# ma921/SOBER

Measured on AMD Instinct MI355X. Metric: recombination-step candidates/sec (N_rec=100000, N_nys=500, d=10, batch=100), higher is better.
Workload: dtype f64

## Files before the change

sober_amd/csrc/chol.hip:

```cpp
#include "common.hpp"
#include "internal.hpp"

namespace sober {

constexpr int CH_NB = 32;
constexpr int CH_T = 512;
constexpr int CH_LDPP = CH_NB + 4;
constexpr int CH_MAXN = 536;

typedef double ch_double4 __attribute__((ext_vector_type(4)));

constexpr int CH_G = 4;
__device__ double ch_sink[CH_T];
#ifdef CM_STAMPS
__device__ double ch_dbg[2];
#endif

__device__ __forceinline__ double ch_rdlane(double v, int l) {
    return __hiloint2double(__builtin_amdgcn_readlane(__double2hiint(v), l),
                            __builtin_amdgcn_readlane(__double2loint(v), l));
}

template <int NC>
__device__ __attribute__((noinline)) void ch_diag_block_n(double* __restrict__ D, double* __restrict__ Xs, double* __restrict__ s_dinv,
                                              int* __restrict__ s_fail_p, double* __restrict__ s_minp_p, int nb, int kb,
                                              int lane, double* __restrict__ xout) {
    constexpr int LDP = CH_NB + 1;
    int& s_fail = *s_fail_p;
    double& s_minp = *s_minp_p;

            const int i = lane & (CH_NB - 1);
            const bool xh = lane >= CH_NB;
            double v[CH_NB];
#ifdef CM_STAMPS
            const long long dbg0 = wall_clock64();
#endif
#pragma unroll
            for (int c = 0; c < CH_NB; ++c) {
                double dv = D[i * LDP + c];
                asm volatile("" : "+v"(dv));
                v[c] = (xh | (i >= nb)) ? ((c == i) ? 1.0 : 0.0) : dv;
            }
            const bool xw = xout != nullptr && xh;
            double* xo = xw ? xout + (size_t)(kb / CH_NB) * CH_NB * CH_NB : ch_sink;
            const int xo_ld = xw ? CH_NB : 0, xo_i = xw ? i : lane;
            double* const o_base = xh ? Xs + i : D + i * LDP;
            const int o_step = xh ? LDP : 1;
            int fail = 0;
            double minp = s_minp;
#pragma unroll
            for (int j = 0; j < NC; ++j) {
                const double djj = ch_rdlane(v[j], j);
                const bool live = (j < nb) & (fail == 0);
                minp = live ? fmin(minp, djj) : minp;
                fail = (live & !(djj > 0.0)) ? kb + j + 1 : fail;
                double rinv = __builtin_amdgcn_rsq(djj);
                {
                    double h = 0.5 * rinv, e = fma(-(djj * rinv), h, 0.5);
                    rinv = fma(rinv, e, rinv);
                    h = 0.5 * rinv; e = fma(-(djj * rinv), h, 0.5);
                    rinv = fma(rinv, e, rinv);
                }
                double l = djj * rinv;
                l = fma(fma(-l, l, djj), 0.5 * rinv, l);
                const double sc = v[j] * rinv;
                v[j] = xh ? sc : ((i == j) ? l : ((i > j) ? sc : 0.0));
                o_base[j * o_step] = v[j];
                xo[j * xo_ld + xo_i] = v[j];
#pragma unroll
                for (int c = j + 1; c < NC; ++c) {
                    const double lcj = ch_rdlane(v[j], c);
                    v[c] = fma(-v[j], lcj, v[c]);
                }
            }
#pragma unroll
            for (int j = NC; j < CH_NB; ++j) { o_base[j * o_step] = v[j]; xo[j * xo_ld + xo_i] = v[j]; }
            if (lane == 0) { s_fail = fail; s_minp = minp; }
#ifdef CM_STAMPS
            if (lane == 0) { ch_dbg[0] = (double)(wall_clock64() - dbg0); ch_dbg[1] = 0.0; }
#endif
        }

__device__ __forceinline__ void ch_diag_block(double* __restrict__ D, double* __restrict__ Xs, double* __restrict__ s_dinv,
                                              int* __restrict__ s_fail_p, double* __restrict__ s_minp_p, int nb, int kb,
                                              int lane, double* __restrict__ xout) {
    if (nb <= 8) ch_diag_block_n<8>(D, Xs, s_dinv, s_fail_p, s_minp_p, nb, kb, lane, xout);
    else if (nb <= 16) ch_diag_block_n<16>(D, Xs, s_dinv, s_fail_p, s_minp_p, nb, kb, lane, xout);
    else ch_diag_block_n<CH_NB>(D, Xs, s_dinv, s_fail_p, s_minp_p, nb, kb, lane, xout);
}

constexpr int CH_SMALLN = 120;
template <bool SMALL>
__global__ __launch_bounds__(CH_T) void k_chol(double* __restrict__ A, int n, int ld, double shift,
                                              int32_t* __restrict__ info, double* __restrict__ min_pivot,
                                              const double* __restrict__ src, int lds_src,
                                              const double* __restrict__ shifts, double* __restrict__ xout,
                                              double* __restrict__ ratio_out) {
    extern __shared__ double lds[];
    if (src != nullptr) {
        A += (size_t)blockIdx.x * n * ld;
        info += blockIdx.x;
        if (min_pivot) min_pivot += blockIdx.x;
        shift = shifts[blockIdx.x];
        for (int i = threadIdx.x >> 6; i < n; i += CH_T / 64)
            for (int j = threadIdx.x & 63; j <= i; j += 64) A[(size_t)i * ld + j] = src[(size_t)i * lds_src + j];
        __threadfence_block();
        __syncthreads();
    }
    constexpr int LDP = CH_NB + 1;
    double* D = lds;
    double* Xs = lds + CH_NB * LDP;
    constexpr int LDPP = CH_LDPP;
    double* P = lds + 2 * CH_NB * LDP;
    double* const A_glob = A;
    const int ld_glob = ld;
    double* As = nullptr;
    if constexpr (SMALL) {
        As = P + (size_t)(n > CH_NB ? n - CH_NB : 0) * LDPP;
    }
    __shared__ int s_fail;
    __shared__ double s_minp;
    __shared__ double s_dinv[CH_NB];
    const int tid = threadIdx.x, lane = tid & 63, wave = tid >> 6;
    const int li = lane & 15, lk = lane >> 4;
    if (tid == 0) { s_fail = 0; s_minp = __builtin_inf(); }
    __shared__ double s_dm[CH_T / 64];
    if (ratio_out != nullptr) {
        double dl = -__builtin_inf();
        for (int i = tid; i < n; i += CH_T) dl = fmax(dl, A_glob[(size_t)i * ld_glob + i] + shift);
#pragma unroll
        for (int o = 32; o > 0; o >>= 1) dl = fmax(dl, __shfl_xor(dl, o, 64));
        if (lane == 0) s_dm[wave] = dl;
    }
    __syncthreads();
    bool ahead0 = false;
    if constexpr (SMALL) {
        const int nb0 = min(CH_NB, n);
#pragma unroll
        for (int t = tid; t < CH_NB * CH_NB; t += CH_T) {
            const int i = t >> 5, j = t & 31;
            double v = (i < nb0 && j <= i) ? A_glob[(size_t)i * ld_glob + j] : 0.0;
            if (i == j && i < nb0) v += shift;
            D[i * LDP + j] = v;
        }
        __syncthreads();
        if (wave == 0) {
            ch_diag_block(D, Xs, s_dinv, &s_fail, &s_minp, nb0, 0, lane, xout);
        } else {
            for (int i = wave - 1; i < n; i += CH_T / 64 - 1)
                for (int j = lane; j <= i; j += 64) As[i * (n + 1) + j] = A_glob[(size_t)i * ld_glob + j];
        }
        A = As;
        ld = n + 1;
        __syncthreads();
        ahead0 = true;
    }
#ifdef CH_STAMPS
    long long st_t[5] = {0, 0, 0, 0, 0}, st_last = wall_clock64();
#define CH_STAMP(K) { const long long now_ = wall_clock64(); st_t[K] += now_ - st_last; st_last = now_; }
#else
#define CH_STAMP(K)
#endif

    bool ahead = ahead0;
    for (int kb = 0; kb < n; kb += CH_NB) {
        const int nb = min(CH_NB, n - kb);
        const int nr = n - kb - nb;
        if (!ahead) {
#pragma unroll
            for (int t = tid; t < CH_NB * CH_NB; t += CH_T) {
                const int i = t >> 5, j = t & 31;
                double v = (i < nb && j <= i) ? A[(size_t)(kb + i) * ld + kb + j] : 0.0;
                if (i == j && i < nb) v += shift;
                D[i * LDP + j] = v;
            }
            __syncthreads();
            CH_STAMP(0)
            if (wave == 0) ch_diag_block(D, Xs, s_dinv, &s_fail, &s_minp, nb, kb, lane, xout);
            __syncthreads();
            CH_STAMP(1)
        }
        if (s_fail != 0) break;
#pragma unroll
        for (int t = tid; t < CH_NB * CH_NB; t += CH_T) {
            const int i = t >> 5, j = t & 31;
            if (i < nb && j <= i) A[(size_t)(kb + i) * ld + kb + j] = D[i * LDP + j];
        }
        if (nr == 0) break;
        {
            const int ntile = (nr + 15) / 16;
            double af[8], an[8];
            if (wave < ntile) {
                const double* arow = A + (size_t)(kb + nb + min(wave * 16 + li, nr - 1)) * ld + kb;
#pragma unroll
                for (int u = 0; u < 8; ++u) af[u] = arow[min(4 * u + lk, nb - 1)];
            }
            for (int t = wave; t < ntile; t += CH_T / 64) {
                const int r0 = t * 16;
                {
                    const int tn = min(t + CH_T / 64, ntile - 1);
                    const double* arow = A + (size_t)(kb + nb + min(tn * 16 + li, nr - 1)) * ld + kb;
#pragma unroll
                    for (int u = 0; u < 8; ++u) an[u] = arow[min(4 * u + lk, nb - 1)];
                }
                ch_double4 acc0 = (ch_double4){0.0, 0.0, 0.0, 0.0}, acc1 = acc0;
#pragma unroll
                for (int u = 0; u < 8; ++u) {
                    const int k = 4 * u + lk;
                    const double a = (k < nb) ? af[u] : 0.0;
                    acc0 = __builtin_amdgcn_mfma_f64_16x16x4f64(a, Xs[li * LDP + k], acc0, 0, 0, 0);
                    acc1 = __builtin_amdgcn_mfma_f64_16x16x4f64(a, Xs[(16 + li) * LDP + k], acc1, 0, 0, 0);
                }
#pragma unroll
                for (int r = 0; r < 4; ++r) {
                    const int row = r0 + lk + 4 * r;
                    if (row < nr) {
                        P[row * LDPP + li] = acc0[r];
                        P[row * LDPP + 16 + li] = acc1[r];
                    }
                }
#pragma unroll
                for (int u = 0; u < 8; ++u) af[u] = an[u];
            }
        }
        __syncthreads();
        CH_STAMP(2)
        for (int r = tid >> 5; r < nr; r += CH_T / 32) {
            const int j = tid & 31;
            if (j < nb) A[(size_t)(kb + nb + r) * ld + kb + j] = P[r * LDPP + j];
        }
        {
            const int nt = (nr + 15) / 16;
            const int wv = __builtin_amdgcn_readfirstlane(wave);
            const bool look = nt * (nt + 1) / 2 >= 8;
            const int t_step = look ? (wv == 0 ? 1 : CH_T / 64 - 1) : CH_T / 64;
            const int nt_mine = (look && wv == 0) ? min(nt, 2) : nt;
            int ntr = 0, ntc = look ? (wv == 0 ? 0 : 2 + wv) : wv;
            while (ntc > ntr) { ntc -= ntr + 1; ++ntr; }
            int tr[CH_G], tc[CH_G], trn[CH_G], tcn[CH_G];
            double cv[CH_G][4], cn[CH_G][4];
            double* const a22 = A + (size_t)(kb + nb) * ld + kb + nb;
// ... 277 lines not shown
                unsigned v = 1u;
                if (jf <= jmax) v = cm_poll(rs, fbase + CM_OFF_FP + 4 * (k * CM_G + o));
                if (v != 1u) s_flag = 0xffu;
            }
        };
        auto gather = [&](int t0, int nthr) {
            for (int cb = k + 1; cb <= jmax; cb += 8)
                for (int gi = t0; gi < CH_NB * CH_NB / 2; gi += nthr) {
                    const int i = gi >> 4, j = (gi & 15) * 2;
                    ch_u32x4 v[8];
#pragma unroll
                    for (int q = 0; q < 8; ++q) {
                        const int c = cb + q, row = min(CH_NB * c + i, n - 1);
                        if (c <= jmax && cm_owner(c) != g)
                            v[q] = __builtin_amdgcn_raw_buffer_load_b128(ra, (unsigned)(((size_t)row * ld + kb + j) * 8), 0, 16);
                    }
#pragma unroll
                    for (int q = 0; q < 8; ++q) {
                        const int c = cb + q, row = CH_NB * c + i;
                        if (c <= jmax && cm_owner(c) != g && row < n) {
                            double* pr = P + (size_t)(row - kb - CH_NB) * LDPP + j;
                            pr[0] = __hiloint2double((int)v[q].y, (int)v[q].x);
                            pr[1] = __hiloint2double((int)v[q].w, (int)v[q].z);
                        }
                    }
                }
        };
        auto walk = [&](int cs0, int wslot, int nwalk) {
            int cs = cs0, ct = wslot;
                int tr[CH_G], tc[CH_G], trn[CH_G], tcn[CH_G];
                double cv[CH_G][4], cn[CH_G][4];
#define CM_TAKE(R, C)                                                                           \
                { while (cs < n_strips && ct > strip_r0(cs) / 16) { ct -= strip_r0(cs) / 16 + 1; ++cs; }   \
                  R = cs < n_strips ? strip_r0(cs) : -1; C = cs < n_strips ? 16 * ct : 0; ct += nwalk; }
#define CM_LOAD(DST, R, C)                                                                      \
                _Pragma("unroll") for (int e = 0; e < 4; ++e)                                   \
                    DST[e] = a22[(size_t)min(max(R, 0) + lk + 4 * e, nr - 1) * ld + min((C) + li, nr - 1)];
#pragma unroll
                for (int q = 0; q < CH_G; ++q) { CM_TAKE(tr[q], tc[q]) CM_LOAD(cv[q], tr[q], tc[q]) }
                while (tr[0] >= 0) {
#pragma unroll
                    for (int q = 0; q < CH_G; ++q) { CM_TAKE(trn[q], tcn[q]) CM_LOAD(cn[q], trn[q], tcn[q]) }
                    ch_double4 acc[CH_G][2];
#pragma unroll
                    for (int q = 0; q < CH_G; ++q) {
                        acc[q][0] = (ch_double4){0.0, 0.0, 0.0, 0.0};
                        acc[q][1] = acc[q][0];
                        const int pa = min(max(tr[q], 0) + li, nr - 1), pb = min(tc[q] + li, nr - 1);
#pragma unroll
                        for (int u = 0; u < 8; u += 2) {
                            acc[q][0] = __builtin_amdgcn_mfma_f64_16x16x4f64(P[pa * LDPP + 4 * u + lk], P[pb * LDPP + 4 * u + lk], acc[q][0], 0, 0, 0);
                            acc[q][1] = __builtin_amdgcn_mfma_f64_16x16x4f64(P[pa * LDPP + 4 * u + 4 + lk], P[pb * LDPP + 4 * u + 4 + lk], acc[q][1], 0, 0, 0);
                        }
                    }
#pragma unroll
                    for (int q = 0; q < CH_G; ++q)
#pragma unroll
                        for (int e = 0; e < 4; ++e) {
                            const int row = tr[q] + lk + 4 * e, col = tc[q] + li;
                            double* dst = (tr[q] >= 0 && row < nr && col <= row) ? a22 + (size_t)row * ld + col : ch_sink + tid;
                            *dst = cv[q][e] - (acc[q][0][e] + acc[q][1][e]);
                        }
#pragma unroll
                    for (int q = 0; q < CH_G; ++q) {
                        tr[q] = trn[q]; tc[q] = tcn[q];
#pragma unroll
                        for (int e = 0; e < 4; ++e) cv[q][e] = cn[q][e];
                    }
                }
#undef CM_TAKE
#undef CM_LOAD
        };
        if (!look) {
            poll_others(tid);
            __syncthreads();
            CM_STAMP(2)
            if (s_flag != 0xffu) gather(tid, CH_T);
            __syncthreads();
            CM_STAMP(3)
            if (s_flag != 0xffu) walk(0, wave, CH_T / 64);
        } else if (wave == 0) {
            __builtin_amdgcn_s_setprio(3);
            const int R0[3] = {0, 16, 16}, C0[3] = {0, 0, 16};
            double cv[3][4];
#pragma unroll
            for (int q = 0; q < 3; ++q)
#pragma unroll
                for (int e = 0; e < 4; ++e)
                    cv[q][e] = a22[(size_t)min(R0[q] + lk + 4 * e, nr - 1) * ld + min(C0[q] + li, nr - 1)];
#pragma unroll
            for (int q = 0; q < 3; ++q) {
                ch_double4 acc0 = (ch_double4){0.0, 0.0, 0.0, 0.0}, acc1 = acc0;
                const int pa = min(R0[q] + li, nr - 1), pb = min(C0[q] + li, nr - 1);
#pragma unroll
                for (int u = 0; u < 8; u += 2) {
                    acc0 = __builtin_amdgcn_mfma_f64_16x16x4f64(P[pa * LDPP + 4 * u + lk], P[pb * LDPP + 4 * u + lk], acc0, 0, 0, 0);
                    acc1 = __builtin_amdgcn_mfma_f64_16x16x4f64(P[pa * LDPP + 4 * u + 4 + lk], P[pb * LDPP + 4 * u + 4 + lk], acc1, 0, 0, 0);
                }
#pragma unroll
                for (int e = 0; e < 4; ++e) {
                    const int row = R0[q] + lk + 4 * e, col = C0[q] + li;
                    double* dst = (row < nr && col <= row) ? a22 + (size_t)row * ld + col : ch_sink + tid;
                    *dst = cv[q][e] - (acc0[e] + acc1[e]);
                }
            }
            __builtin_amdgcn_s_waitcnt(0);
            const int kb2 = kb + CH_NB, nb2 = min(CH_NB, n - kb2);
#pragma unroll
            for (int t = lane; t < CH_NB * CH_NB; t += 64) {
                const int i = t >> 5, j = t & 31;
                double v = (i < nb2 && j <= i) ? A[(size_t)(kb2 + i) * ld + kb2 + j] : 0.0;
                if (i == j && i < nb2) v += shift;
                D[i * LDP + j] = v;
            }
            __builtin_amdgcn_wave_barrier();
            ch_diag_block(D, Xs, s_dinv, &s_fail, &s_minp, nb2, kb2, lane, nullptr);
            __builtin_amdgcn_s_setprio(0);
        } else {
            if (wave == 1) poll_others(lane);
            sub_barrier();
            if (s_flag != 0xffu) gather(tid - 64, CH_T - 64);
            sub_barrier();
            if (s_flag != 0xffu) walk(2, wave - 1, CH_T / 64 - 1);
        }
        CM_STAMP(4)
        ahead = look;
        __threadfence_block();
        __syncthreads();
        CM_STAMP(5)
        if (s_flag == 0xffu) {
            if (tid == 0) {
                __builtin_amdgcn_raw_buffer_store_b32(1, rs, CM_OFF_ERR, 0, 16);
                info[rung] = CM_INFO_EXCHANGE;
            }
            break;
        }
    }
#ifdef CM_STAMPS
    if (tid == 0 && n >= 480) { for (int q = 0; q < 6; ++q) A[(size_t)g * ld + 400 + q] = (double)cs_t[q]; A[(size_t)g * ld + 410] = ch_dbg[0]; A[(size_t)g * ld + 411] = ch_dbg[1]; }
#endif
    if (verdict >= 0 && tid == 0) {
        double mp = s_minp;
        for (int q = 0; q < verdict; ++q) {
            const unsigned lo = (unsigned)__builtin_amdgcn_raw_buffer_load_b32(rs, fbase + CM_OFF_MP + 8 * q, 0, 16);
            const unsigned hi = (unsigned)__builtin_amdgcn_raw_buffer_load_b32(rs, fbase + CM_OFF_MP + 8 * q + 4, 0, 16);
            mp = fmin(mp, __hiloint2double((int)hi, (int)lo));
        }
        info[rung] = s_fail;
        if (min_pivot) min_pivot[rung] = mp;
    }
}

constexpr int TB_WAVES = 2;
__global__ __launch_bounds__(TB_WAVES * 64) void k_trsm_blocks(const double* __restrict__ Y, int64_t m, int q, int ldy,
                                                              const double* __restrict__ L, int ldl,
                                                              const double* __restrict__ Xinv,
                                                              double* __restrict__ Q, int ldq) {
    extern __shared__ double tb_lds[];
    const int lane = threadIdx.x & 63, wave = threadIdx.x >> 6;
    const int li = lane & 15, lk = lane >> 4;
    const int qpad = ((q + 31) / 32) * 32, LS = qpad + 4;
    double* stash = tb_lds + (size_t)wave * (16 * LS + 16 * 36);
    double* tbuf = stash + 16 * LS;
    const int64_t R0 = ((int64_t)blockIdx.x * TB_WAVES + wave) * 16;
    if (R0 >= m) return;
    const int nblk = qpad / 32;
    for (int jb = 0; jb < nblk; ++jb) {
        const int c0 = 32 * jb;
        ch_double4 acc[2];
#pragma unroll
        for (int jt = 0; jt < 2; ++jt)
#pragma unroll
            for (int r = 0; r < 4; ++r) {
                const int64_t row = min(R0 + lk + 4 * r, m - 1);
                const int col = c0 + 16 * jt + li;
                const double v = Y[row * ldy + min(col, q - 1)];
                acc[jt][r] = (col < q) ? v : 0.0;
            }
        for (int kb = 0; kb < jb; ++kb) {
#pragma unroll
            for (int u = 0; u < 8; ++u) {
                const int kc = 32 * kb + 4 * u + lk;
                const double a = -stash[li * LS + kc];
#pragma unroll
                for (int jt = 0; jt < 2; ++jt) {
                    const int lr = c0 + 16 * jt + li;
                    const double b = L[(size_t)min(lr, q - 1) * ldl + kc];
                    acc[jt] = __builtin_amdgcn_mfma_f64_16x16x4f64(a, (lr < q) ? b : 0.0, acc[jt], 0, 0, 0);
                }
            }
        }
#pragma unroll
        for (int jt = 0; jt < 2; ++jt)
#pragma unroll
            for (int r = 0; r < 4; ++r) tbuf[(lk + 4 * r) * 36 + 16 * jt + li] = acc[jt][r];
        __builtin_amdgcn_wave_barrier();
        const double* X = Xinv + (size_t)jb * 32 * 32;
        ch_double4 out[2] = {(ch_double4){0.0, 0.0, 0.0, 0.0}, (ch_double4){0.0, 0.0, 0.0, 0.0}};
#pragma unroll
        for (int u = 0; u < 8; ++u) {
            const double a = tbuf[li * 36 + 4 * u + lk];
#pragma unroll
            for (int jt = 0; jt < 2; ++jt)
                out[jt] = __builtin_amdgcn_mfma_f64_16x16x4f64(a, X[(16 * jt + li) * 32 + 4 * u + lk], out[jt], 0, 0, 0);
        }
        __builtin_amdgcn_wave_barrier();
#pragma unroll
        for (int jt = 0; jt < 2; ++jt)
#pragma unroll
            for (int r = 0; r < 4; ++r) {
                const int64_t row = R0 + lk + 4 * r;
                const int col = c0 + 16 * jt + li;
                stash[(lk + 4 * r) * LS + col] = out[jt][r];
                if (row < m && col < q) Q[row * ldq + col] = out[jt][r];
            }
        __builtin_amdgcn_wave_barrier();
    }
}

__global__ __launch_bounds__(256) void k_abs_sym(const double* __restrict__ C, int n, int ld,
                                                 double* __restrict__ out, int ldo, int32_t* __restrict__ flag,
                                                 unsigned long long* __restrict__ dmax_bits) {
    __shared__ double tm[32][33];
    const int tx = threadIdx.x & 31, ty = threadIdx.x >> 5;
    const int i0 = blockIdx.y * 32, j0 = blockIdx.x * 32;
    for (int r = ty; r < 32; r += 8) {
        const int i = j0 + r, j = i0 + tx;
        tm[r][tx] = (i < n && j < n) ? C[(size_t)i * ld + j] : 0.0;
    }
    __syncthreads();
    bool asym = false;
    const double big = 1.7976931348623157e308;
    for (int r = ty; r < 32; r += 8) {
        const int i = i0 + r, j = j0 + tx;
        if (i < n && j < n) {
            double a = C[(size_t)i * ld + j], b = tm[tx][r];
            asym |= !(a == b);
            a = (a != a) ? 0.0 : fmin(fmax(a, -big), big);
            b = (b != b) ? 0.0 : fmin(fmax(b, -big), big);
            const double v = sqrt(a * b);
            out[(size_t)i * ldo + j] = v;
            if (dmax_bits != nullptr && i == j) atomicMax(dmax_bits, (unsigned long long)__double_as_longlong(v));
        }
    }
    if (__syncthreads_or(asym) && threadIdx.x == 0) atomicOr(flag, 1);
}

__global__ void k_jitter_ladder(double* __restrict__ A, int n, int ld, int k) {
    const int i = blockIdx.x * blockDim.x + threadIdx.x;
    if (i >= n) return;
    double d = A[(size_t)i * ld + i], jit = 1e-5;
    for (int t = 0; t < k; ++t) { d = __dadd_rn(d, jit); jit = __dmul_rn(jit, 2.0); }
    A[(size_t)i * ld + i] = d;
}

__global__ void k_jitter_ladder_auto(double* __restrict__ A, int n, int ld, const int32_t* __restrict__ info,
                                     int n_rungs, int32_t* __restrict__ k_out) {
    const int j = blockIdx.x * blockDim.x + threadIdx.x, i = blockIdx.y;
    int k = 0;
    while (k < n_rungs && info[k] != 0) ++k;
    if (i == 0 && j == 0) *k_out = k;
    if (j >= n) return;
    if (i == j) {
        double d = A[(size_t)i * ld + i], jit = 1e-5;
        for (int t = 0; t < k; ++t) { d = __dadd_rn(d, jit); jit = __dmul_rn(jit, 2.0); }
        A[(size_t)i * ld + i] = d;
    } else if (k == n_rungs) {
        A[(size_t)i * ld + j] = 0.0;
    }
}

}

namespace sober {
__global__ void k_probe_mc_init(uint32_t* __restrict__ ws, int64_t n_words, int32_t* __restrict__ info, int n_info, int32_t value,
                                uint32_t* __restrict__ pre, int64_t n_pre) {
    const int64_t t = (int64_t)blockIdx.x * blockDim.x + threadIdx.x;
    if (t < n_words) ws[t] = 0u;
    if (pre != nullptr) {
        const int64_t i0 = (uint32_t*)info - pre;
        if (t < n_pre && !(t >= i0 && t < i0 + n_info)) pre[t] = 0u;
    }
    if (t < n_info) info[t] = value;
}
}

namespace sober {
constexpr int CB_MAXN = 2048;
constexpr int CB_TILE = 64;

__global__ __launch_bounds__(256) void k_cb_init(double* __restrict__ work, int n, const double* __restrict__ src, int ld_src,
                                                 int32_t* __restrict__ info, double* __restrict__ min_pivot, int n_rungs) {
    const int i = blockIdx.x, rung = blockIdx.y;
    double* A = work + (size_t)rung * n * n;
    for (int c = threadIdx.x; c <= i; c += 256) A[(size_t)i * n + c] = src[(size_t)i * ld_src + c];
    if (i == 0 && threadIdx.x == 0) { info[rung] = 0; if (min_pivot) min_pivot[rung] = __builtin_inf(); }
}

__global__ __launch_bounds__(64) void k_cb_diag(double* __restrict__ work, int n, int kb, const double* __restrict__ shifts,
                                                double* __restrict__ xinv, int32_t* __restrict__ info,
                                                double* __restrict__ min_pivot) {
    constexpr int LDP = CH_NB + 1;
    __shared__ double D[CH_NB * LDP], Xs[CH_NB * LDP], s_dinv[CH_NB];
    __shared__ int s_fail;
    __shared__ double s_minp;
    const int rung = blockIdx.x, lane = threadIdx.x;
    double* A = work + (size_t)rung * n * n;
    const int nb = min(CH_NB, n - kb);
    const double shift = shifts[rung];
#pragma unroll
    for (int t = lane; t < CH_NB * CH_NB; t += 64) {
        const int i = t >> 5, j = t & 31;
        double v = (i < nb && j <= i) ? A[(size_t)(kb + i) * n + kb + j] : 0.0;
        if (i == j && i < nb) v += shift;
        D[i * LDP + j] = v;
    }
    if (lane == 0) { s_fail = 0; s_minp = __builtin_inf(); }
// ... 13 lines not shown
    constexpr int LDP = CH_NB + 1, LDPP = CH_LDPP;
    __shared__ double Xs[CH_NB * LDP], Pr[CB_TILE * LDPP], Pc[CB_TILE * LDPP];
    const int rung = blockIdx.y, tid = threadIdx.x, lane = tid & 63, wave = tid >> 6;
    const int li = lane & 15, lk = lane >> 4;
    double* A = work + (size_t)rung * n * n;
    const int base = kb + CH_NB;
    int bi = 0, rest = blockIdx.x;
    while (rest > bi) { rest -= bi + 1; ++bi; }
    const int bj = rest;
    const int R0 = base + CB_TILE * bi, C0 = base + CB_TILE * bj;
    const double* xi = xinv + (size_t)rung * CH_NB * CH_NB;
    for (int t = tid; t < CH_NB * CH_NB; t += 256) Xs[(t >> 5) * LDP + (t & 31)] = xi[t];
    __syncthreads();
#pragma unroll
    for (int side = 0; side < 2; ++side) {
        if (side == 1 && bi == bj) break;
        const int r0 = (side == 0 ? R0 : C0) + 16 * wave;
        const double* arow = A + (size_t)min(r0 + li, n - 1) * n + kb;
        double af[8];
#pragma unroll
        for (int u = 0; u < 8; ++u) af[u] = arow[4 * u + lk];
        ch_double4 acc0 = (ch_double4){0.0, 0.0, 0.0, 0.0}, acc1 = acc0;
#pragma unroll
        for (int u = 0; u < 8; ++u) {
            const int k = 4 * u + lk;
            acc0 = __builtin_amdgcn_mfma_f64_16x16x4f64(af[u], Xs[li * LDP + k], acc0, 0, 0, 0);
            acc1 = __builtin_amdgcn_mfma_f64_16x16x4f64(af[u], Xs[(16 + li) * LDP + k], acc1, 0, 0, 0);
        }
        double* P = side == 0 ? Pr : Pc;
#pragma unroll
        for (int r = 0; r < 4; ++r) {
            const int row = 16 * wave + lk + 4 * r;
            P[row * LDPP + li] = acc0[r];
            P[row * LDPP + 16 + li] = acc1[r];
        }
    }
    __syncthreads();
    const double* Pcol = (bi == bj) ? Pr : Pc;
#pragma unroll
    for (int ct = 0; ct < 4; ++ct) {
        if (bi == bj && ct > wave) break;
        double cv[4];
#pragma unroll
        for (int e = 0; e < 4; ++e)
            cv[e] = A[(size_t)min(R0 + 16 * wave + lk + 4 * e, n - 1) * n + min(C0 + 16 * ct + li, n - 1)];
        ch_double4 acc0 = (ch_double4){0.0, 0.0, 0.0, 0.0}, acc1 = acc0;
        const int pa = 16 * wave + li, pb = 16 * ct + li;
#pragma unroll
        for (int u = 0; u < 8; u += 2) {
            acc0 = __builtin_amdgcn_mfma_f64_16x16x4f64(Pr[pa * LDPP + 4 * u + lk], Pcol[pb * LDPP + 4 * u + lk], acc0, 0, 0, 0);
            acc1 = __builtin_amdgcn_mfma_f64_16x16x4f64(Pr[pa * LDPP + 4 * u + 4 + lk], Pcol[pb * LDPP + 4 * u + 4 + lk], acc1, 0, 0, 0);
        }
#pragma unroll
        for (int e = 0; e < 4; ++e) {
            const int row = R0 + 16 * wave + lk + 4 * e, col = C0 + 16 * ct + li;
            if (row < n && col <= row) A[(size_t)row * n + col] = cv[e] - (acc0[e] + acc1[e]);
        }
    }
}
}

namespace sober {
__global__ void k_orth_merge(int32_t* __restrict__ info, double* __restrict__ piv, double* __restrict__ ratio,
                             const int32_t* __restrict__ info2, const double* __restrict__ piv2, const double* __restrict__ ratio2) {
    if (threadIdx.x != 0 || blockIdx.x != 0) return;
    if (*info == 0) *info = *info2;
    *piv = fmin(*piv, *piv2);
    if (*piv2 != *piv2) *piv = *piv2;
    if (ratio != nullptr) {
        *ratio = fmin(*ratio, *ratio2);
        if (*ratio2 != *ratio2) *ratio = *ratio2;
    }
}
}
int sober::orth_merge(int32_t* info, double* piv, double* ratio, const int32_t* info2, const double* piv2, const double* ratio2,
                      void* stream) {
    if (!info || !piv || !info2 || !piv2 || (ratio && !ratio2)) return SOBER_E_ARG;
    hipLaunchKernelGGL(sober::k_orth_merge, dim3(1), dim3(64), 0, (hipStream_t)stream, info, piv, ratio, info2, piv2, ratio2);
    LAUNCH_CHECK();
    return 0;
}

extern "C" int sober_nystrom_max_n(void) { return sober::CB_MAXN; }

extern "C" int sober_cholesky_probe_batched(const double* src, int n, int ld_src, const double* shifts, int n_shifts,
                                            double* work, int32_t* info, double* min_pivot, void* xinv_ws,
                                            int64_t ws_bytes, void* stream) {
    if (!src || !shifts || !work || !info || !xinv_ws || n <= 0 || ld_src < n || n_shifts <= 0) return SOBER_E_ARG;
    if (n > sober::CB_MAXN || n_shifts > 64) return SOBER_E_DIM;
    if (ws_bytes < (int64_t)n_shifts * sober::CH_NB * sober::CH_NB * 8) return SOBER_E_WS;
    hipStream_t st = (hipStream_t)stream;
    hipLaunchKernelGGL(sober::k_cb_init, dim3(n, n_shifts), dim3(256), 0, st, work, n, src, ld_src, info, min_pivot, n_shifts);
    LAUNCH_CHECK();
    for (int kb = 0; kb < n; kb += sober::CH_NB) {
        hipLaunchKernelGGL(sober::k_cb_diag, dim3(n_shifts), dim3(64), 0, st, work, n, kb, shifts, (double*)xinv_ws, info,
                           min_pivot);
        LAUNCH_CHECK();
        const int rest = n - kb - sober::CH_NB;
        if (rest <= 0) break;
        const int T = (rest + sober::CB_TILE - 1) / sober::CB_TILE;
        hipLaunchKernelGGL(sober::k_cb_update, dim3(T * (T + 1) / 2, n_shifts), dim3(256), 0, st, work, n, kb,
                           (const double*)xinv_ws);
        LAUNCH_CHECK();
    }
    return 0;
}

namespace sober {
}

extern "C" int sober_chol_max_n(void) { return sober::CH_MAXN; }

extern "C" int sober_cholesky_inv_ratio(double* A, int n, int ld, double shift, int32_t* info, double* min_pivot,
                                        double* xinv, double* ratio_out, void* stream);
extern "C" int sober_cholesky_inv(double* A, int n, int ld, double shift, int32_t* info, double* min_pivot,
                                  double* xinv, void* stream) {
    return sober_cholesky_inv_ratio(A, n, ld, shift, info, min_pivot, xinv, nullptr, stream);
}

extern "C" int sober_cholesky_inv_ratio(double* A, int n, int ld, double shift, int32_t* info, double* min_pivot,
                                        double* xinv, double* ratio_out, void* stream) {
    if (!A || !info || n <= 0 || ld < n) return SOBER_E_ARG;
    if (n > sober::CH_MAXN) return SOBER_E_DIM;
    const int nr = n > sober::CH_NB ? n - sober::CH_NB : 0;
    size_t bytes = ((size_t)2 * sober::CH_NB * (sober::CH_NB + 1) + (size_t)nr * sober::CH_LDPP) * sizeof(double);
    static std::atomic<unsigned long long> attr_set{0};
    if (sober_attr_needed(attr_set)) {
        HIP_TRY(hipFuncSetAttribute((const void*)sober::k_chol<false>, hipFuncAttributeMaxDynamicSharedMemorySize,
                                    160 * 1024 - 512));
        HIP_TRY(hipFuncSetAttribute((const void*)sober::k_chol<true>, hipFuncAttributeMaxDynamicSharedMemorySize,
                                    160 * 1024 - 512));
        sober_attr_done(attr_set);
    }
    if (n <= sober::CH_SMALLN) {
        bytes += (size_t)n * (n + 1) * sizeof(double);
        hipLaunchKernelGGL(sober::k_chol<true>, dim3(1), dim3(sober::CH_T), bytes, (hipStream_t)stream, A, n, ld, shift,
                           info, min_pivot, (const double*)nullptr, 0, (const double*)nullptr, xinv, ratio_out);
    } else {
        hipLaunchKernelGGL(sober::k_chol<false>, dim3(1), dim3(sober::CH_T), bytes, (hipStream_t)stream, A, n, ld, shift,
                           info, min_pivot, (const double*)nullptr, 0, (const double*)nullptr, xinv, ratio_out);
    }
    LAUNCH_CHECK();
    return 0;
}

extern "C" int sober_cholesky(double* A, int n, int ld, double shift, int32_t* info, double* min_pivot,
                              void* stream) {
    return sober_cholesky_inv(A, n, ld, shift, info, min_pivot, nullptr, stream);
}

extern "C" int sober_trsm_blocks(const double* Y, int64_t m, int q, int ldy, const double* L, int ldl,
                                 const double* Xinv, double* Q, int ldq, void* stream) {
    if (!Y || !L || !Xinv || !Q || m <= 0 || q <= 0 || q > sober::CH_MAXN || ldy < q || ldl < q || ldq < q) return SOBER_E_ARG;
    const int qpad = ((q + 31) / 32) * 32;
    const size_t bytes = (size_t)sober::TB_WAVES * (16 * (qpad + 4) + 16 * 36) * sizeof(double);
    static std::atomic<unsigned long long> attr_set{0};
    if (sober_attr_needed(attr_set)) {
        HIP_TRY(hipFuncSetAttribute((const void*)sober::k_trsm_blocks, hipFuncAttributeMaxDynamicSharedMemorySize,
                                    160 * 1024 - 512));
        sober_attr_done(attr_set);
    }
    const int64_t row_blocks = (m + 15) / 16;
    hipLaunchKernelGGL(sober::k_trsm_blocks, dim3((unsigned)((row_blocks + sober::TB_WAVES - 1) / sober::TB_WAVES)),
                       dim3(sober::TB_WAVES * 64), bytes, (hipStream_t)stream, Y, m, q, ldy, L, ldl, Xinv, Q, ldq);
    LAUNCH_CHECK();
    return 0;
}

extern "C" int sober_cholesky_probe_piv(const double* src, int n, int ld_src, const double* shifts, int n_shifts,
                                        double* work, int32_t* info, double* min_pivot, void* stream);
extern "C" int sober_cholesky_probe(const double* src, int n, int ld_src, const double* shifts, int n_shifts,
                                    double* work, int32_t* info, void* stream) {
    return sober_cholesky_probe_piv(src, n, ld_src, shifts, n_shifts, work, info, nullptr, stream);
}

extern "C" int sober_cholesky_probe_piv(const double* src, int n, int ld_src, const double* shifts, int n_shifts,
                                        double* work, int32_t* info, double* min_pivot, void* stream) {
    if (!src || !shifts || !work || !info || n <= 0 || ld_src < n || n_shifts <= 0) return SOBER_E_ARG;
    if (n > sober::CH_MAXN) return SOBER_E_DIM;
    const int nr = n > sober::CH_NB ? n - sober::CH_NB : 0;
    const size_t bytes = ((size_t)2 * sober::CH_NB * (sober::CH_NB + 1) + (size_t)nr * sober::CH_LDPP) * sizeof(double);
    HIP_TRY(hipFuncSetAttribute((const void*)sober::k_chol<false>, hipFuncAttributeMaxDynamicSharedMemorySize,
                                160 * 1024 - 512));
    hipLaunchKernelGGL(sober::k_chol<false>, dim3(n_shifts), dim3(sober::CH_T), bytes, (hipStream_t)stream, work, n, n, 0.0,
                       info, min_pivot, src, ld_src, shifts, (double*)nullptr, (double*)nullptr);
    LAUNCH_CHECK();
    return 0;
}

extern "C" int64_t sober_cholesky_probe_mc_ws_bytes(int n, int n_shifts) {
    if (n <= 0 || n_shifts <= 0 || n_shifts > 16 || n > sober::CH_MAXN) return 0;
    const int64_t flags = ((int64_t)sober::CM_HDR + (int64_t)n_shifts * sober::CM_RUNG_BYTES + 255) / 256 * 256;
    return flags + (int64_t)n_shifts * sober::CM_MAXB * sober::CH_NB * sober::CH_NB * 8;
}

int64_t sober::probe_mc_flag_bytes(int n_shifts) {
    return ((int64_t)sober::CM_HDR + (int64_t)n_shifts * sober::CM_RUNG_BYTES + 255) / 256 * 256;
}

int sober::nystrom_flags_init(void* flags_block, int64_t flags_bytes, void* probe_ws, int64_t ws_flag_bytes, int32_t* info,
                              int n_info, void* stream) {
    if (!flags_block || !probe_ws || !info || flags_bytes <= 0 || (flags_bytes & 3) || ws_flag_bytes <= 0 || n_info <= 0)
        return SOBER_E_ARG;
    const int64_t n_pre = flags_bytes / 4, n_ws = ws_flag_bytes / 4;
    const int64_t n = n_pre > n_ws ? n_pre : n_ws;
    hipLaunchKernelGGL(sober::k_probe_mc_init, dim3((unsigned)((n + 255) / 256)), dim3(256), 0, (hipStream_t)stream,
                       (uint32_t*)probe_ws, n_ws, info, n_info, (int32_t)sober::CM_INFO_EXCHANGE, (uint32_t*)flags_block, n_pre);
    LAUNCH_CHECK();
    return 0;
}

int sober::cholesky_probe_mc(const double* src, int n, int ld_src, const double* shifts, int n_shifts, double* work,
                             int32_t* info, double* min_pivot, void* ws, int64_t ws_bytes, bool init, void* stream) {
    if (!src || !shifts || !work || !info || !ws || n <= 0 || ld_src < n || n_shifts <= 0) return SOBER_E_ARG;
    if (n > sober::CH_MAXN || n_shifts > 16) return SOBER_E_DIM;
    const int64_t need = sober_cholesky_probe_mc_ws_bytes(n, n_shifts);
    if (ws_bytes < need || need > 0x7fffffff) return SOBER_E_WS;
    const int64_t flags = sober::probe_mc_flag_bytes(n_shifts);
    const int nr = n > sober::CH_NB ? n - sober::CH_NB : 0;
    const size_t bytes = ((size_t)2 * sober::CH_NB * (sober::CH_NB + 1) + (size_t)nr * sober::CH_LDPP) * sizeof(double);
    static std::atomic<unsigned long long> attr_set{0};
    if (sober_attr_needed(attr_set)) {
        HIP_TRY(hipFuncSetAttribute((const void*)sober::k_chol_mc, hipFuncAttributeMaxDynamicSharedMemorySize,
                                    160 * 1024 - 512));
        sober_attr_done(attr_set);
    }
    if (init) {
        hipLaunchKernelGGL(sober::k_probe_mc_init, dim3((unsigned)((flags / 4 + 255) / 256)), dim3(256), 0, (hipStream_t)stream,
                           (uint32_t*)ws, (int64_t)(flags / 4), info, n_shifts, (int32_t)sober::CM_INFO_EXCHANGE,
                           (uint32_t*)nullptr, (int64_t)0);
        LAUNCH_CHECK();
    }
    const size_t lds_bytes = bytes > (size_t)84 * 1024 ? bytes : (size_t)84 * 1024;
    hipLaunchKernelGGL(sober::k_chol_mc, dim3(256), dim3(sober::CH_T), lds_bytes, (hipStream_t)stream, work, n, n, info,
                       min_pivot, src, ld_src, shifts, n_shifts, (unsigned char*)ws, (unsigned)need, (unsigned)flags);
    LAUNCH_CHECK();
    return 0;
}

extern "C" int sober_cholesky_probe_mc(const double* src, int n, int ld_src, const double* shifts, int n_shifts,
                                       double* work, int32_t* info, double* min_pivot, void* ws, int64_t ws_bytes,
                                       void* stream) {
    return sober::cholesky_probe_mc(src, n, ld_src, shifts, n_shifts, work, info, min_pivot, ws, ws_bytes, true, stream);
}

extern "C" int sober_abs_sym_dmax(const double* C, int n, int ld, double* out, int ldo, int32_t* flag, double* dmax,
                                  void* stream) {
    if (!C || !out || !flag || n <= 0 || ld < n || ldo < n || n > 65535) return SOBER_E_ARG;
    hipLaunchKernelGGL(sober::k_abs_sym, dim3((n + 31) / 32, (n + 31) / 32), dim3(256), 0, (hipStream_t)stream, C, n,
                       ld, out, ldo, flag, (unsigned long long*)dmax);
    LAUNCH_CHECK();
    return 0;
}

extern "C" int sober_abs_sym(const double* C, int n, int ld, double* out, int ldo, int32_t* flag, void* stream) {
    return sober_abs_sym_dmax(C, n, ld, out, ldo, flag, nullptr, stream);
}

extern "C" int sober_jitter_ladder(double* A, int n, int ld, int k, void* stream) {
    if (!A || n <= 0 || ld < n || k < 0) return SOBER_E_ARG;
    if (k == 0) return 0;
    hipLaunchKernelGGL(sober::k_jitter_ladder, dim3((n + 255) / 256), dim3(256), 0, (hipStream_t)stream, A, n, ld, k);
    LAUNCH_CHECK();
    return 0;
}

extern "C" int sober_jitter_ladder_auto(double* A, int n, int ld, const int32_t* info, int n_rungs, int32_t* k_out,
                                        void* stream) {
    if (!A || !info || !k_out || n <= 0 || ld < n || n_rungs <= 0) return SOBER_E_ARG;
    hipLaunchKernelGGL(sober::k_jitter_ladder_auto, dim3((n + 255) / 256, n), dim3(256), 0, (hipStream_t)stream, A, n,
                       ld, info, n_rungs, k_out);
    LAUNCH_CHECK();
    return 0;
}
```

Measured before the change: 27.57 million.

## Split Cholesky diagonal block into halves with MFMA update; stage TRSM operands in LDS

The 32-wide diagonal-block factorization is split into two 16-column halves. The trailing-half update and the inverse-block off-diagonal product are done with f64 MFMA instructions, replacing the serial readlane-based rank-1 updates over all 32 columns. Separately, the blocked TRSM kernel gets templated fast paths for up to four 32-column blocks (q up to 128). These paths preload the Y rows into registers and stage the Xinv and L blocks once per workgroup in LDS, instead of reading them from global memory per wave. This adds LDS footprint and register pressure, along with more template instantiations.

```diff
diff --git a/sober_amd/csrc/chol.hip b/sober_amd/csrc/chol.hip
--- a/sober_amd/csrc/chol.hip
+++ b/sober_amd/csrc/chol.hip
@@ -19,6 +19,36 @@
 __device__ __forceinline__ double ch_rdlane(double v, int l) {
     return __hiloint2double(__builtin_amdgcn_readlane(__double2hiint(v), l),
                             __builtin_amdgcn_readlane(__double2loint(v), l));
+}
+
+template <int J0, int J1>
+__device__ __forceinline__ void ch_diag_cols(double (&v)[CH_NB], int i, bool xh, double* o_base, int o_step, double* xo, int xo_ld,
+                                             int xo_i, int nb, int kb, int& fail, double& minp) {
+#pragma unroll
+    for (int j = J0; j < J1; ++j) {
+        const double djj = ch_rdlane(v[j], j);
+        const bool live = (j < nb) & (fail == 0);
+        minp = live ? fmin(minp, djj) : minp;
+        fail = (live & !(djj > 0.0)) ? kb + j + 1 : fail;
+        double rinv = __builtin_amdgcn_rsq(djj);
+        {
+            double h = 0.5 * rinv, e = fma(-(djj * rinv), h, 0.5);
+            rinv = fma(rinv, e, rinv);
+            h = 0.5 * rinv; e = fma(-(djj * rinv), h, 0.5);
+            rinv = fma(rinv, e, rinv);
+        }
+        double l = djj * rinv;
+        l = fma(fma(-l, l, djj), 0.5 * rinv, l);
+        const double sc = v[j] * rinv;
+        v[j] = xh ? sc : ((i == j) ? l : ((i > j) ? sc : 0.0));
+        o_base[j * o_step] = v[j];
+        xo[j * xo_ld + xo_i] = v[j];
+#pragma unroll
+        for (int c = j + 1; c < J1; ++c) {
+            const double lcj = ch_rdlane(v[j], c);
+            v[c] = fma(-v[j], lcj, v[c]);
+        }
+    }
 }
 
 template <int NC>
@@ -48,31 +78,7 @@
             const int o_step = xh ? LDP : 1;
             int fail = 0;
             double minp = s_minp;
-#pragma unroll
-            for (int j = 0; j < NC; ++j) {
-                const double djj = ch_rdlane(v[j], j);
-                const bool live = (j < nb) & (fail == 0);
-                minp = live ? fmin(minp, djj) : minp;
-                fail = (live & !(djj > 0.0)) ? kb + j + 1 : fail;
-                double rinv = __builtin_amdgcn_rsq(djj);
-                {
-                    double h = 0.5 * rinv, e = fma(-(djj * rinv), h, 0.5);
-                    rinv = fma(rinv, e, rinv);
-                    h = 0.5 * rinv; e = fma(-(djj * rinv), h, 0.5);
-                    rinv = fma(rinv, e, rinv);
-                }
-                double l = djj * rinv;
-                l = fma(fma(-l, l, djj), 0.5 * rinv, l);
-                const double sc = v[j] * rinv;
-                v[j] = xh ? sc : ((i == j) ? l : ((i > j) ? sc : 0.0));
-                o_base[j * o_step] = v[j];
-                xo[j * xo_ld + xo_i] = v[j];
-#pragma unroll
-                for (int c = j + 1; c < NC; ++c) {
-                    const double lcj = ch_rdlane(v[j], c);
-                    v[c] = fma(-v[j], lcj, v[c]);
-                }
-            }
+            ch_diag_cols<0, NC>(v, i, xh, o_base, o_step, xo, xo_ld, xo_i, nb, kb, fail, minp);
 #pragma unroll
             for (int j = NC; j < CH_NB; ++j) { o_base[j * o_step] = v[j]; xo[j * xo_ld + xo_i] = v[j]; }
             if (lane == 0) { s_fail = fail; s_minp = minp; }
@@ -81,12 +87,73 @@
 #endif
         }
 
+__device__ __attribute__((noinline)) void ch_diag_block_halves(double* __restrict__ D, double* __restrict__ Xs,
+                                                               int* __restrict__ s_fail_p, double* __restrict__ s_minp_p, int nb,
+                                                               int kb, int lane, double* __restrict__ xout) {
+    constexpr int LDP = CH_NB + 1, H = CH_NB / 2;
+    const int i = lane & (CH_NB - 1), li = lane & 15, lk = lane >> 4;
+    const bool xh = lane >= CH_NB;
+    double v[CH_NB];
+#ifdef CM_STAMPS
+    const long long dbg0 = wall_clock64();
+#endif
+#pragma unroll
+    for (int c = 0; c < CH_NB; ++c) {
+        double dv = c < H ? D[i * LDP + c] : 0.0;
+        asm volatile("" : "+v"(dv));
+        v[c] = (xh | (i >= nb) | (c >= H)) ? ((c == i) ? 1.0 : 0.0) : dv;
+    }
+    const bool xw = xout != nullptr && xh;
+    double* const xblk = xout != nullptr ? xout + (size_t)(kb / CH_NB) * CH_NB * CH_NB : nullptr;
+    double* const o_base = xh ? Xs + i : D + i * LDP;
+    const int o_step = xh ? LDP : 1;
+    int fail = 0;
+    double minp = *s_minp_p;
+    ch_diag_cols<0, H>(v, i, xh, o_base, o_step, xw ? xblk : ch_sink, xw ? CH_NB : 0, xw ? i : lane, nb, kb, fail, minp);
+    __builtin_amdgcn_wave_barrier();
+    double a[4];
+#pragma unroll
+    for (int u = 0; u < 4; ++u) a[u] = D[(H + li) * LDP + 4 * u + lk];
+    ch_double4 acc = (ch_double4){0.0, 0.0, 0.0, 0.0}, t = acc;
+#pragma unroll
+    for (int u = 0; u < 4; ++u) acc = __builtin_amdgcn_mfma_f64_16x16x4f64(a[u], a[u], acc, 0, 0, 0);
+#pragma unroll
+    for (int r = 0; r < 4; ++r) {
+        double* p = D + (H + lk + 4 * r) * LDP + H + li;
+        *p = *p - acc[r];
+    }
+#pragma unroll
+    for (int u = 0; u < 4; ++u) t = __builtin_amdgcn_mfma_f64_16x16x4f64(a[u], Xs[(4 * u + lk) * LDP + li], t, 0, 0, 0);
+    __builtin_amdgcn_wave_barrier();
+#pragma unroll
+    for (int c = H; c < CH_NB; ++c) {
+        double dv = D[i * LDP + c];
+        asm volatile("" : "+v"(dv));
+        v[c] = (xh | (i >= nb)) ? v[c] : dv;
+    }
+    const bool xw2 = xw && i >= H;
+    ch_diag_cols<H, CH_NB>(v, i, xh, o_base, o_step, xw2 ? xblk : ch_sink, xw2 ? CH_NB : 0, xw2 ? i : lane, nb, kb, fail, minp);
+    __builtin_amdgcn_wave_barrier();
+    ch_double4 o = (ch_double4){0.0, 0.0, 0.0, 0.0};
+#pragma unroll
+    for (int u = 0; u < 4; ++u) o = __builtin_amdgcn_mfma_f64_16x16x4f64(-Xs[(H + li) * LDP + H + lk + 4 * u], t[u], o, 0, 0, 0);
+#pragma unroll
+    for (int r = 0; r < 4; ++r) {
+        Xs[(H + lk + 4 * r) * LDP + li] = o[r];
+        if (xblk != nullptr) xblk[(H + lk + 4 * r) * CH_NB + li] = o[r];
+    }
+    if (lane == 0) { *s_fail_p = fail; *s_minp_p = minp; }
+#ifdef CM_STAMPS
+    if (lane == 0) { ch_dbg[0] = (double)(wall_clock64() - dbg0); ch_dbg[1] = 0.0; }
+#endif
+}
+
 __device__ __forceinline__ void ch_diag_block(double* __restrict__ D, double* __restrict__ Xs, double* __restrict__ s_dinv,
                                               int* __restrict__ s_fail_p, double* __restrict__ s_minp_p, int nb, int kb,
                                               int lane, double* __restrict__ xout) {
     if (nb <= 8) ch_diag_block_n<8>(D, Xs, s_dinv, s_fail_p, s_minp_p, nb, kb, lane, xout);
     else if (nb <= 16) ch_diag_block_n<16>(D, Xs, s_dinv, s_fail_p, s_minp_p, nb, kb, lane, xout);
-    else ch_diag_block_n<CH_NB>(D, Xs, s_dinv, s_fail_p, s_minp_p, nb, kb, lane, xout);
+    else ch_diag_block_halves(D, Xs, s_fail_p, s_minp_p, nb, kb, lane, xout);
 }
 
 constexpr int CH_SMALLN = 120;
@@ -670,6 +737,9 @@
 }
 
 constexpr int TB_WAVES = 2;
+constexpr int TB_LDB = 36;
+constexpr int TB_FAST_NB = 4;
+template <int NB>
 __global__ __launch_bounds__(TB_WAVES * 64) void k_trsm_blocks(const double* __restrict__ Y, int64_t m, int q, int ldy,
                                                               const double* __restrict__ L, int ldl,
                                                               const double* __restrict__ Xinv,
@@ -681,6 +751,104 @@
     double* stash = tb_lds + (size_t)wave * (16 * LS + 16 * 36);
     double* tbuf = stash + 16 * LS;
     const int64_t R0 = ((int64_t)blockIdx.x * TB_WAVES + wave) * 16;
+    if constexpr (NB > 0) {
+        constexpr int NP = NB * (NB - 1) / 2;
+        constexpr int PER = 32 * 32 / (TB_WAVES * 64);
+        double* Xl = tb_lds + (size_t)TB_WAVES * (16 * LS + 16 * 36);
+        double* Ll = Xl + NB * 32 * TB_LDB;
+        const bool mine = R0 < m;
+        double yv[NB][2][4];
+        if (mine) {
+#pragma unroll
+            for (int jb = 0; jb < NB; ++jb)
+#pragma unroll
+                for (int jt = 0; jt < 2; ++jt)
+#pragma unroll
+                    for (int r = 0; r < 4; ++r) {
+                        const int64_t row = min(R0 + lk + 4 * r, m - 1);
+                        const int col = 32 * jb + 16 * jt + li;
+                        const double v = Y[row * ldy + min(col, q - 1)];
+                        yv[jb][jt][r] = (col < q) ? v : 0.0;
+                    }
+        }
+        double xv[NB][PER], lv[NP > 0 ? NP : 1][PER];
+#pragma unroll
+        for (int b = 0; b < NB; ++b)
+#pragma unroll
+            for (int e = 0; e < PER; ++e) xv[b][e] = Xinv[(size_t)b * 1024 + e * (TB_WAVES * 64) + threadIdx.x];
+#pragma unroll
+        for (int jb = 1; jb < NB; ++jb)
+#pragma unroll
+            for (int kb = 0; kb < jb; ++kb)
+#pragma unroll
+                for (int e = 0; e < PER; ++e) {
+                    const int t = e * (TB_WAVES * 64) + threadIdx.x, lr = 32 * jb + (t >> 5);
+                    const double v = L[(size_t)min(lr, q - 1) * ldl + 32 * kb + (t & 31)];
+                    lv[jb * (jb - 1) / 2 + kb][e] = (lr < q) ? v : 0.0;
+                }
+#pragma unroll
+        for (int b = 0; b < NB; ++b)
+#pragma unroll
+            for (int e = 0; e < PER; ++e) {
+                const int t = e * (TB_WAVES * 64) + threadIdx.x;
+                Xl[b * 32 * TB_LDB + (t >> 5) * TB_LDB + (t & 31)] = xv[b][e];
+            }
+#pragma unroll
+        for (int p = 0; p < NP; ++p)
+#pragma unroll
+            for (int e = 0; e < PER; ++e) {
+                const int t = e * (TB_WAVES * 64) + threadIdx.x;
+                Ll[p * 32 * TB_LDB + (t >> 5) * TB_LDB + (t & 31)] = lv[p][e];
+            }
+        __syncthreads();
+        if (!mine) return;
+#pragma unroll
+        for (int jb = 0; jb < NB; ++jb) {
+            const int c0 = 32 * jb;
+            ch_double4 acc[2];
+#pragma unroll
+            for (int jt = 0; jt < 2; ++jt)
+#pragma unroll
+                for (int r = 0; r < 4; ++r) acc[jt][r] = yv[jb][jt][r];
+#pragma unroll
+            for (int kb = 0; kb < jb; ++kb) {
+                const double* Lb = Ll + (jb * (jb - 1) / 2 + kb) * 32 * TB_LDB;
+#pragma unroll
+                for (int u = 0; u < 8; ++u) {
+                    const double a = -stash[li * LS + 32 * kb + 4 * u + lk];
+#pragma unroll
+                    for (int jt = 0; jt < 2; ++jt)
+                        acc[jt] = __builtin_amdgcn_mfma_f64_16x16x4f64(a, Lb[(16 * jt + li) * TB_LDB + 4 * u + lk], acc[jt], 0, 0, 0);
+                }
+            }
+#pragma unroll
+            for (int jt = 0; jt < 2; ++jt)
+#pragma unroll
+                for (int r = 0; r < 4; ++r) tbuf[(lk + 4 * r) * 36 + 16 * jt + li] = acc[jt][r];
+            __builtin_amdgcn_wave_barrier();
+            const double* X = Xl + jb * 32 * TB_LDB;
+            ch_double4 out[2] = {(ch_double4){0.0, 0.0, 0.0, 0.0}, (ch_double4){0.0, 0.0, 0.0, 0.0}};
+#pragma unroll
+            for (int u = 0; u < 8; ++u) {
+                const double a = tbuf[li * 36 + 4 * u + lk];
+#pragma unroll
+                for (int jt = 0; jt < 2; ++jt)
+                    out[jt] = __builtin_amdgcn_mfma_f64_16x16x4f64(a, X[(16 * jt + li) * TB_LDB + 4 * u + lk], out[jt], 0, 0, 0);
+            }
+            __builtin_amdgcn_wave_barrier();
+#pragma unroll
+            for (int jt = 0; jt < 2; ++jt)
+#pragma unroll
+                for (int r = 0; r < 4; ++r) {
+                    const int64_t row = R0 + lk + 4 * r;
+                    const int col = c0 + 16 * jt + li;
+                    stash[(lk + 4 * r) * LS + col] = out[jt][r];
+                    if (row < m && col < q) Q[row * ldq + col] = out[jt][r];
+                }
+            __builtin_amdgcn_wave_barrier();
+        }
+        return;
+    }
     if (R0 >= m) return;
     const int nblk = qpad / 32;
     for (int jb = 0; jb < nblk; ++jb) {
@@ -1000,16 +1168,23 @@
 extern "C" int sober_trsm_blocks(const double* Y, int64_t m, int q, int ldy, const double* L, int ldl,
                                  const double* Xinv, double* Q, int ldq, void* stream) {
     if (!Y || !L || !Xinv || !Q || m <= 0 || q <= 0 || q > sober::CH_MAXN || ldy < q || ldl < q || ldq < q) return SOBER_E_ARG;
-    const int qpad = ((q + 31) / 32) * 32;
-    const size_t bytes = (size_t)sober::TB_WAVES * (16 * (qpad + 4) + 16 * 36) * sizeof(double);
+    const int qpad = ((q + 31) / 32) * 32, nblk = qpad / 32;
+    const int nb = nblk <= sober::TB_FAST_NB ? nblk : 0;
+    const size_t bytes = ((size_t)sober::TB_WAVES * (16 * (qpad + 4) + 16 * 36) +
+                          (size_t)(nb + nb * (nb - 1) / 2) * 32 * sober::TB_LDB) * sizeof(double);
+    static_assert(sober::TB_FAST_NB == 4, "one instantiation per block count below");
+    using kern_t = void (*)(const double*, int64_t, int, int, const double*, int, const double*, double*, int);
+    static const kern_t kerns[sober::TB_FAST_NB + 1] = {sober::k_trsm_blocks<0>, sober::k_trsm_blocks<1>, sober::k_trsm_blocks<2>,
+                                                       sober::k_trsm_blocks<3>, sober::k_trsm_blocks<4>};
     static std::atomic<unsigned long long> attr_set{0};
     if (sober_attr_needed(attr_set)) {
-        HIP_TRY(hipFuncSetAttribute((const void*)sober::k_trsm_blocks, hipFuncAttributeMaxDynamicSharedMemorySize,
-                                    160 * 1024 - 512));
+        for (const kern_t k : kerns)
+            HIP_TRY(hipFuncSetAttribute((const void*)k, hipFuncAttributeMaxDynamicSharedMemorySize,
+                                        160 * 1024 - 512));
         sober_attr_done(attr_set);
     }
     const int64_t row_blocks = (m + 15) / 16;
-    hipLaunchKernelGGL(sober::k_trsm_blocks, dim3((unsigned)((row_blocks + sober::TB_WAVES - 1) / sober::TB_WAVES)),
+    hipLaunchKernelGGL(kerns[nb], dim3((unsigned)((row_blocks + sober::TB_WAVES - 1) / sober::TB_WAVES)),
                        dim3(sober::TB_WAVES * 64), bytes, (hipStream_t)stream, Y, m, q, ldy, L, ldl, Xinv, Q, ldq);
     LAUNCH_CHECK();
     return 0;
```

Result: no change. 27.68 million (median of 3 runs) (+0.4%).
